# pmorenoz/HetMOGP

Measured on AMD Instinct MI355X. Metric: ELBO-steps/sec (one step = ELBO + all parameter gradients), higher is better.
Workload: dtype f64

## Files before the change

### hetmogp_amd/csrc/common.h

```cpp
#pragma once
#include <hip/hip_runtime.h>
#include <stdint.h>
#include <string>

#define HMOGP_WAVE 64
#ifndef HMOGP_POTRF_NB
#define HMOGP_POTRF_NB 32
#endif

typedef double f64x4 __attribute__((ext_vector_type(4)));
typedef double f64x2 __attribute__((ext_vector_type(2)));

struct HipError {
  hipError_t code;
  const char* what;
  const char* file;
  int line;
};
#define HIP_TRY(expr)                                          \
  do {                                                         \
    hipError_t _e = (expr);                                    \
    if (_e != hipSuccess) throw HipError{_e, #expr, __FILE__, __LINE__}; \
  } while (0)

__device__ __forceinline__ double wave_sum(double v) {
#pragma unroll
  for (int o = 32; o > 0; o >>= 1) v += __shfl_xor(v, o, 64);
  return v;
}

__device__ __forceinline__ double block_sum(double v, double* scratch) {
  v = wave_sum(v);
  const int lane = threadIdx.x & 63, w = threadIdx.x >> 6, nw = (blockDim.x + 63) >> 6;
  __syncthreads();
  if (lane == 0) scratch[w] = v;
  __syncthreads();
  double r = 0.0;
  if (threadIdx.x == 0)
    for (int i = 0; i < nw; ++i) r += scratch[i];
  return r;
}

struct GemmArgs {
  const double* A = nullptr;
  const double* B = nullptr;
  double* C = nullptr;
  const double* kscale = nullptr;
  int M = 0, N = 0, K = 0;
  int lda = 0, ldb = 0, ldc = 0;
  long long sA = 0, sB = 0, sC = 0, sS = 0;
  double alpha = 1.0, beta = 0.0;
  int nbatch = 1;
  int M_last = 0, N_last = 0, K_last = 0;
  int nouter = 1;
  long long oA = 0, oB = 0, oC = 0, oS = 0;
  int ksplit = 1;
  long long sSplit = 0;
  int a_kmajor = 0, b_kmajor = 1;
  int lower_only = 0;
  int diag_balance = 1;
  int role = 0;
  double* fs_part = nullptr;
  const double* fs_a = nullptr;
  const double* fs_x = nullptr;
  const double* fs_z = nullptr;
  const double* fs_ell = nullptr;
  int fs_ldz = 0, fs_P = 1, fs_hyper = 0;
  long long fs_sPart = 0, fs_sA = 0, fs_sZ = 0;
  int store_c = 1;
  int fs_sq = 0;
  const double* fs_k = nullptr;
  const double* c_src = nullptr;
  int c_sub = 0;
  int a_tri = 0, b_tri = 0;
  const int* win = nullptr;
  long long win_stride = 0;
};
void launch_combine_parts(const double* part, int tiles, long long n, double* p, double* c, double* pt, double* ct,
                          hipStream_t s, int nb = 1, long long sPart = 0, long long ldn = 0);
void launch_gemm_f64(const GemmArgs& g, hipStream_t stream);
bool gemm_rowpass_eligible(const GemmArgs& g);
void launch_gemm_rowpass(const GemmArgs& g, hipStream_t stream);
int launch_gemm_rowpass_or_general(const GemmArgs& g, hipStream_t stream);
bool gemm_rowpass_would_take(const GemmArgs& g);
constexpr int GEMM_MAX_FWD_PARTS = 4;
bool gemm_small_eligible(const GemmArgs& g);
void launch_gemm_small(const GemmArgs& g, hipStream_t stream);

void launch_potrf_batched(double* A, int Q, int M, int* d_info, double* dscr, hipStream_t stream, int panel_begin = 0,
                          int panel_end = -1);
void launch_trtri_batched(const double* L, double* Linv, double* tmp, int Q, int M, hipStream_t stream, bool linv_is_zero = false);
void launch_ltl_batched(const double* Linv, double* Out, int Q, int M, hipStream_t stream);

void launch_fill(double* p, long long n, double v, hipStream_t stream);
void launch_unpack_tril(const double* L_flat , double* L , int Q, int M, hipStream_t s);
void launch_gemv_batched(const double* A, const double* x, double* y, int Q, int M, long long sx, int incx,
                         hipStream_t s);
```

### hetmogp_amd/csrc/engine.hip

```cpp
#include "engine_impl.h"

hipEvent_t hmogp_engine::new_event() {
  if (pool_used == pool.size()) {
    hipEvent_t e;
    HIP_TRY(hipEventCreate(&e));
    pool.push_back(e);
  }
  return pool[pool_used++];
}

void hmogp_engine::collect_spans() {
  static const bool dbg = getenv("HMOGP_DEBUG_TIMELINE") != nullptr;
  for (auto& s : spans) {
    float f = 0.f;
    if (hipEventElapsedTime(&f, s.a, s.b) == hipSuccess) ms[s.cat] += f;
    if (dbg) {
      float t0 = 0.f;
      if (hipEventElapsedTime(&t0, ev_begin0, s.a) == hipSuccess)
        std::fprintf(stderr, "[hmogp timeline] cat %d  start %9.3f ms  dur %9.3f ms\n", s.cat, t0, f);
    }
  }
  spans.clear();
  pool_used = 0;
}

hmogp_engine::~hmogp_engine() {
  drop_graphs();
  comm_destroy();
  for (auto e : pool) (void)hipEventDestroy(e);
  if (h_info2) (void)hipHostFree(h_info2);
  if (ev_ng) (void)hipEventDestroy(ev_ng);
  if (h_small) (void)hipHostFree(h_small);
  for (auto e : {ev_begin0, ev_begin1, ev_fin0, ev_fin1, ev_fork, ev_gsk, ev_zero, ev_info, ev_S, ev_join, ev_col, ev_kuf, ev_params, ev_ua, ev_qu})
    if (e) (void)hipEventDestroy(e);
  if (hstage) (void)hipHostFree(hstage);
  if (h_info) (void)hipHostFree(h_info);
  if (h_cond) (void)hipHostFree(h_cond);
  if (ev_cond) (void)hipEventDestroy(ev_cond);
  if (st2_own) (void)hipStreamDestroy(st2_own);
  if (st3_own) (void)hipStreamDestroy(st3_own);
  if (st) (void)hipStreamDestroy(st);
}

void hmogp_engine::init(const hmogp_config* c) {
  if (!c || c->abi_version != HMOGP_ABI_VERSION) throw EngineError{HMOGP_E_INVALID, "bad config / ABI version"};
  T = c->T, Q = c->Q, M = c->M, P = c->P, Df = c->Df, device = c->device;
  if (T < 1 || Q < 1 || M < 1 || Df < 1) throw EngineError{HMOGP_E_INVALID, "T, Q, M, Df must be >= 1"};
  if (P < 1 || P > 4) throw EngineError{HMOGP_E_INVALID, "input dimension P must be 1..4"};
  if (Q > HMOGP_MAXQ) throw EngineError{HMOGP_E_INVALID, "Q exceeds HMOGP_MAXQ (8)"};
  if (c->chunk_rows > 0) {
    chunk = c->chunk_rows;
  } else {
    const long long fit = (64LL << 30) / (16LL * Q * M);
    chunk = std::max<long long>(4096, std::min<long long>(1048576, fit / 1024 * 1024));
  }
  use_windows = (c->flags & HMOGP_CFG_EXACT_ZERO_WINDOWS) != 0;
  cache_kuu = (c->flags & HMOGP_CFG_CACHE_KUU) != 0;
  no_small = (c->flags & HMOGP_CFG_NO_SMALL_PATH) != 0;
  strict = strict_cfg = (c->flags & HMOGP_CFG_STRICT_QF) != 0;
  if (strict && use_windows) throw EngineError{HMOGP_E_INVALID, "HMOGP_CFG_STRICT_QF and HMOGP_CFG_EXACT_ZERO_WINDOWS exclude each other"};
  if (c->flags & ~(HMOGP_CFG_EXACT_ZERO_WINDOWS | HMOGP_CFG_CACHE_KUU | HMOGP_CFG_NO_SMALL_PATH | HMOGP_CFG_STRICT_QF))
    throw EngineError{HMOGP_E_INVALID, "unknown bits in hmogp_config.flags"};
  quirks = c->quirks;
  if (quirks & ~HMOGP_QUIRKS_REFERENCE) throw EngineError{HMOGP_E_INVALID, "unknown bits in hmogp_config.quirks"};
  if (use_windows && M > 8192) throw EngineError{HMOGP_E_INVALID, "exact-zero windows support M <= 8192"};
  int ndev = 0;
  if (hipGetDeviceCount(&ndev) != hipSuccess || ndev < 1)
    throw EngineError{HMOGP_E_NO_DEVICE, "no HIP device visible (this library has no CPU path)"};
  if (device < 0 || device >= ndev) throw EngineError{HMOGP_E_NO_DEVICE, "HIP device ordinal out of range"};
  HIP_TRY(hipSetDevice(device));
  {
    int lo = 0, hi = 0;
    HIP_TRY(hipDeviceGetStreamPriorityRange(&lo, &hi));
    HIP_TRY(hipStreamCreateWithPriority(&st, hipStreamNonBlocking, hi));
    const char* cus_env = getenv("HMOGP_ST2_CUS");
    int cus = cus_env ? atoi(cus_env) : 0;
    hipDeviceProp_t prop;
    HIP_TRY(hipGetDeviceProperties(&prop, device));
    if (cus > 0 && cus < prop.multiProcessorCount) {
      std::vector<uint32_t> mask((prop.multiProcessorCount + 31) / 32, 0u);
      for (int i = 0; i < cus; ++i) mask[i / 32] |= 1u << (i % 32);
      if (hipExtStreamCreateWithCUMask(&st2, (uint32_t)mask.size(), mask.data()) != hipSuccess) st2 = nullptr;
    }
    const char* free_env = getenv("HMOGP_ST2_FREE");
    const int nfree = free_env ? atoi(free_env) : 0;
    if (!st2 && nfree > 0 && nfree < 32 && prop.multiProcessorCount == 256) {
      const char* lay = getenv("HMOGP_ST2_LAYOUT");
      const int layout = lay ? atoi(lay) : 1;
      st2_masked = true;
      std::vector<uint32_t> mask(8, 0xFFFFFFFFu);
      for (int x = 0; x < 8; ++x)
        for (int c = 32 - nfree; c < 32; ++c) {
          const int bit = layout == 0 ? x * 32 + c : c * 8 + x;
          mask[bit / 32] &= ~(1u << (bit % 32));
        }
      if (hipExtStreamCreateWithCUMask(&st2, (uint32_t)mask.size(), mask.data()) != hipSuccess) st2 = nullptr, st2_masked = false;
    }
    if (!st2) HIP_TRY(hipStreamCreateWithPriority(&st2, hipStreamNonBlocking, lo));
    HIP_TRY(hipStreamCreateWithPriority(&st3, hipStreamNonBlocking, hi));
    st2_own = st2, st3_own = st3;
  }
  for (hipEvent_t* e : {&ev_fork, &ev_gsk, &ev_zero, &ev_info, &ev_S, &ev_join, &ev_col, &ev_kuf, &ev_params, &ev_ua, &ev_qu})
    HIP_TRY(hipEventCreateWithFlags(e, hipEventDisableTiming));
  HIP_TRY(hipEventRecord(ev_qu, st));
  HIP_TRY(hipEventRecord(ev_join, st));
  for (hipEvent_t* e : {&ev_begin0, &ev_begin1, &ev_fin0, &ev_fin1}) HIP_TRY(hipEventCreate(e));
  f_index.assign(c->f_index, c->f_index + Df);
  d_index.assign(c->d_index, c->d_index + Df);
  tasks.resize(T);
  int d = 0;
  for (int t = 0; t < T; ++t) {
    Task& k = tasks[t];
    k.lik = c->lik_id[t];
    k.param = c->lik_param ? c->lik_param[t] : 0.0;
    if (k.lik == HMOGP_LIK_GAUSSIAN && !(k.param > 0.0)) k.param = 0.5;
    k.dimf = lik_dimf(k.lik, k.param);
    check_lik_param(k.lik, k.param);
    k.qparam = k.lik == HMOGP_LIK_ORDINAL ? ordinal_table(k.param).sigma : k.param;
    if (k.dimf < 1 || k.dimf > HMOGP_MAXJ) throw EngineError{HMOGP_E_INVALID, "unsupported likelihood / dim_f"};
    k.d0 = d;
    for (int j = 0; j < k.dimf; ++j, ++d)
      if (d >= Df || f_index[d] != t || d_index[d] != j)
        throw EngineError{HMOGP_E_INVALID, "f_index / d_index inconsistent with the likelihood list"};
  }
  if (d != Df) throw EngineError{HMOGP_E_INVALID, "Df does not match the likelihood list"};
  const long long MM = (long long)M * M;
  NG = 2 + Df;
  oR = MM, oDZ = MM + M, oSA = oDZ + (long long)M * P, oSL = oSA + 1, oSWK = oSA + 2;
  per_q = oSWK + Df;
  nstats = NG + Q * per_q;
  stats.ensure(sizeof(double) * nstats, true);
  nwire = NG + Q * ((long long)M * (M + 1) / 2 + (per_q - MM));
  for (int t = 0; t < T; ++t) {
    Task& k = tasks[t];
    const int J = k.dimf;
    k.nscal = 2 + 2 * Q + J + Q * J;
    std::vector<long long> off(k.nscal);
    off[0] = 0, off[1] = 1;
    for (int q = 0; q < Q; ++q) {
      off[2 + 2 * q] = NG + q * per_q + oSA;
      off[3 + 2 * q] = NG + q * per_q + oSL;
      for (int j = 0; j < J; ++j) off[2 + 2 * Q + J + q * J + j] = NG + q * per_q + oSWK + k.d0 + j;
    }
    for (int j = 0; j < J; ++j) off[2 + 2 * Q + j] = 2 + k.d0 + j;
    k.offsets.ensure(sizeof(long long) * k.nscal);
    HIP_TRY(hipMemcpy(k.offsets.p, off.data(), sizeof(long long) * k.nscal, hipMemcpyHostToDevice));
  }
  const size_t mmq = sizeof(double) * MM * Q;
  for (DevBuf* b : {&Kuu, &Luu, &Kuui, &L, &S, &KiS, &KSK, &C, &Ctri, &Sqi, &tmpA, &tmpB, &HK, &G, &GSK, &dKmm, &dLdS}) b->ensure(mmq, true);
  oJit = 2 * Q + 2 * Q * Df, oW0 = oJit + Q, oBs = oW0 + Q * Df, oSeq = oBs + T;
  n_small = oSeq + 1;
  auto even = [](long long n) { return (n + 1) & ~1LL; };
  const long long nZ = (long long)M * Q * P, nmu = (long long)M * Q, nL = ((long long)M * (M + 1) / 2) * Q;
  oZ = even(n_small), oMu = oZ + even(nZ), oLf = oMu + even(nmu), n_params = oLf + even(nL);
  dparams.ensure(sizeof(double) * n_params);
// ... 448 lines not shown
```

### hetmogp_amd/csrc/engine_impl.h

```cpp
#pragma once
#include <algorithm>
#include <cmath>
#include <cstdio>
#include <cstdlib>
#include <cstring>
#include <string>
#include <vector>

#include <chrono>
#include <thread>

#include <dlfcn.h>
#include <hip/hip_runtime.h>
extern "C" {
typedef struct ncclComm* ncclComm_t;
}
namespace hm_nccl {
struct UniqueId { char internal[128]; };
enum : int { Success = 0, InProgress = 7, DataDouble = 8, OpSum = 0 };
using GetUniqueId = int (*)(UniqueId*);
using CommInitRank = int (*)(ncclComm_t*, int, UniqueId, int);
using CommDestroy = int (*)(ncclComm_t);
using CommAbort = int (*)(ncclComm_t);
using CommGetAsyncError = int (*)(ncclComm_t, int*);
// ... 166 lines not shown
  double* h_small = nullptr;
  long long n_small = 0, oZ = 0, oMu = 0, oLf = 0, n_params = 0, oJit = 0, oW0 = 0, oBs = 0, oSeq = 0;
  int eval_seq = 0;
  DevBuf Kuu, Luu, Kuui, L, S, KiS, KSK, C, Ctri, Sqi, tmpA, tmpB, HK, G, GSK, dKmm, dLdS;
  DevBuf a, Kr, gmu, gL, klout, rowout, dinfo, djit, dscr;
  long long ws_rows = 0;
  DevBuf Kh, Pt, vp, vc, vpt, vct, valpha, vbeta, valpha0, vbeta0;
  DevBuf colred;
  DevBuf stats, wire, slabs, colpart, quadpart, fwdpart, winrow, wincol, winhit, Xws, dstage;
  long long nwire = 0;
  int* h_info = nullptr;
  double* hstage = nullptr;
  size_t hstage_cap = 0;
  bool began = false, evaluated = false;
  bool qu_resident = false;
  DevBuf ad_gms_m, ad_sms_m, ad_step_m, ad_pend_m, ad_gms_L, ad_sms_L, ad_step_L, ad_pend_L;

  struct Span {
    hipEvent_t a, b;
    int cat;
  };
  std::vector<hipEvent_t> pool;
  size_t pool_used = 0;
  std::vector<Span> spans;
  double ms[NCAT] = {0};
  long long launches[NCAT] = {0};
  hipEvent_t ev_begin0 = nullptr, ev_begin1 = nullptr, ev_fin0 = nullptr, ev_fin1 = nullptr;
  bool st2_masked = false;
  hipStream_t st2_own = nullptr, st3_own = nullptr;
  bool small_mode = false;
  bool small_path = false, small_veto = false, small_info_pending = false, info_early = false;
  double* hstage_dev = nullptr;
  bool small_rows = false;
  DevBuf smallslab;
  struct RetryRegular {};
  struct SmallGraph {
    std::vector<long long> key;
    hipGraph_t graph = nullptr;
    hipGraphExec_t exec = nullptr;
  };
  std::vector<SmallGraph> graphs;
  std::vector<std::vector<long long>> warm_keys;
  long long graph_replays = 0, graph_captures = 0;
  void drop_graphs(bool keep_warm = false);
  std::vector<long long> graph_key(const hmogp_params* p) const;
  bool graph_step(const hmogp_params* p, hmogp_outputs* out);
  bool graphs_broken = false, via_graph = false;
  std::vector<long long> pending_warm;
  void mark_warm();
  hipStream_t st2 = nullptr;
  hipStream_t st3 = nullptr;
  hipEvent_t ev_qu = nullptr;
  hipEvent_t ev_fork = nullptr, ev_gsk = nullptr, ev_zero = nullptr, ev_info = nullptr, ev_S = nullptr, ev_join = nullptr, ev_col = nullptr, ev_kuf = nullptr, ev_params = nullptr,
             ev_ua = nullptr;

  hipEvent_t new_event();
  struct Scope {
    hmogp_engine* e;
    Span s;
    hipStream_t stream;
    bool on_;
    Scope(hmogp_engine* eng, int cat, int nlaunch, hipStream_t on = nullptr) : e(eng), stream(on ? on : eng->st) {
      static const bool off = getenv("HMOGP_NO_SPANS") != nullptr;
      on_ = !off && (!eng->small_mode || cat == CAT_EXCHANGE);
      s.cat = cat;
      e->launches[cat] += nlaunch;
      if (!on_) return;
      s.a = e->new_event();
      s.b = e->new_event();
      (void)hipEventRecord(s.a, stream);
    }
    ~Scope() {
      if (!on_) return;
      (void)hipEventRecord(s.b, stream);
      e->spans.push_back(s);
    }
  };
  void collect_spans();

  ncclComm_t comm = nullptr;
  int comm_ranks = 1, comm_rank = 0;
  bool exchanged = false;

  void comm_init(int nranks, int rank, const void* id);
  void comm_destroy();
  void comm_abort();
  void wait_exchanged();
  void exchange();

  ~hmogp_engine();

  double* Hq(int q) { return stats.d() + NG + q * per_q; }

  void init(const hmogp_config* c);

  void set_task_data(int t, const double* X, const double* Y, long long N);

  void ensure_workspace(long long rows);

  long long ws_strict_rows = 0;
  void ensure_strict_workspace();

  void upload_params(const hmogp_params* p, bool enqueue = true);

  void mm(const double* A, bool a_k, const double* B, bool b_k, double* Cc, double alpha = 1.0, long long sA = -1,
          int lda = -1, hipStream_t stream = nullptr, int a_tri = 0, int b_tri = 0, bool lower_only = false) {
    GemmArgs g;
// ... 72 lines not shown
```

### hetmogp_amd/csrc/engine_rows.hip

```cpp
#include "engine_impl.h"

void hmogp_engine::u_algebra_small() {
  Scope sc(this, CAT_MM, 1);
  kuu_key_valid = false;
  if (!h_info) HIP_TRY(hipHostMalloc((void**)&h_info, sizeof(int) * HMOGP_MAXQ, hipHostMallocDefault));
  for (int q = 0; q < Q; ++q)
    if (rung[q] == -2) rung[q] = -1;
  if (!pools.empty()) {
    stage_pool_inputs(pools[0], st);
    if (!small_rows) kuf_pool(pools[0], st);
    kuf_prefetched = true;
    HIP_TRY(hipEventRecord(ev_kuf, st));
  }
  SmallU u;
  u.M = M, u.Q = Q, u.P = P, u.ldz = Q * P;
  u.Z = dZ.d(), u.var = dvar.d(), u.ell = dell.d(), u.jit = dsmall.d() + oJit, u.mu = dmu.d(), u.Lflat = dLflat.d();
  u.Kuu = Kuu.d(), u.Luu = Luu.d(), u.Kuui = Kuui.d(), u.L = L.d(), u.S = S.d(), u.KiS = KiS.d(), u.KSK = KSK.d(), u.C = C.d();
  u.Ctri = Ctri.d(), u.Sqi = Sqi.d(), u.a = a.d(), u.klout = klout.d(), u.info = dinfo.as<int>(), u.flag = dinfo.as<int>() + HMOGP_MAXQ;
  u.seq = dsmall.d() + oSeq;
  u.zero = stats.d(), u.nzero = nstats;
  launch_u_small(u, st);
  if (info_early) HIP_TRY(hipMemcpyAsync(h_info, dinfo.p, sizeof(int) * Q, hipMemcpyDeviceToHost, st));
  small_info_pending = true;
  HIP_TRY(hipEventRecord(ev_join, st));
// ... 216 lines not shown
    Scope sc(this, CAT_FWD, 2);
    GemmArgs g;
    g.A = Ah.d(), g.lda = M, g.a_kmajor = 0, g.sA = sK;
    g.B = Bt, g.ldb = M, g.b_kmajor = 1, g.sB = MM, g.b_tri = +1;
    g.C = Pt.d(), g.ldc = M, g.sC = sK;
    g.M = (int)n, g.N = M, g.K = M;
    g.nbatch = Q;
    g.role = 1;
    const int tiles = (M + 127) / 128;
    g.fs_part = fwdpart.d(), g.fs_sPart = 4LL * FWD_PARTS * tiles * ldn, g.fs_sq = 1, g.store_c = 0;
    static const bool t2_env = [] {
      const char* e = getenv("HMOGP_STRICT_T2");
      return !(e && e[0] == '0');
    }();
    if (t2_env && gemm_rowpass_would_take(g)) {
      const int nparts = launch_gemm_rowpass_or_general(g, st);
      launch_combine_parts(fwdpart.d(), nparts * tiles, n, nullptr, vct.d(), nullptr, nullptr, st, Q, g.fs_sPart, ldn);
      t2_fused = true;
    } else {
      rows_gemm(Ah.d(), Bt, 1, +1, Pt.d());
    }
  }
  StrictRows sr;
  sr.M = M, sr.Q = Q, sr.P = P, sr.ldz = Q * P, sr.n = n, sr.ldn = ldn, sr.sK = sK, sr.sZ = P;
  sr.Kh = Kh.d(), sr.Ah = Ah.d(), sr.Tt = Pt.d(), sr.Pt = Pt.d(), sr.mu = dmu.d(), sr.w3 = strict_two ? nullptr : w3.d(), sr.a = a.d();
  sr.X = X, sr.Z = dZ.d(), sr.ell = dell.d();
  sr.p = vp.d(), sr.c = vc.d(), sr.pg = vpg.d(), sr.cg = vcg.d(), sr.pt = nullptr, sr.ct = nullptr;
  sr.phase = 0;
  sr.t2 = t2_fused ? vct.d() : nullptr;
  {
    Scope sc(this, CAT_STRICT_STATS, 1);
    if (stats_fused && t2_fused)
      launch_trsm_stats_combine(trsmpart.d(), ts.sPart, ldn, 4, n, Q, vct.d(), vp.d(), vc.d(), ldn, st);
    else
      launch_strict_rowstats(sr, st);
  }
  sr.t2 = nullptr;
  if (!grads) return;
  static const bool p1_env = [] {
    const char* e = getenv("HMOGP_STRICT_P1");
    return !(e && e[0] == '0');
  }();
  {
    GemmArgs g;
    g.A = Ah.d(), g.lda = M, g.a_kmajor = 0, g.sA = sK;
    g.B = Bp, g.ldb = M, g.b_kmajor = 1, g.sB = MM;
    g.C = Pt.d(), g.ldc = M, g.sC = sK;
    g.M = (int)n, g.N = M, g.K = M;
    g.nbatch = Q;
    g.role = 1;
    const int tiles = (M + 127) / 128;
    g.fs_part = fwdpart.d(), g.fs_sPart = 4LL * FWD_PARTS * tiles * ldn, g.fs_a = a.d(), g.fs_sA = M, g.fs_k = Kh.d();
    if (p1_env && gemm_rowpass_would_take(g)) {
      {
        Scope sc(this, CAT_FWD, 1);
        launch_gemm_rowpass_or_general(g, st);
      }
      Scope sc(this, CAT_STRICT_STATS, 1);
      launch_combine_parts(fwdpart.d(), 4 * tiles, n, vpg.d(), vcg.d(), nullptr, nullptr, st, Q, g.fs_sPart, ldn);
      return;
    }
  }
  {
    Scope sc(this, CAT_FWD, 1);
    rows_gemm(Ah.d(), Bp, 1, 0, Pt.d());
  }
  Scope sc(this, CAT_STRICT_STATS, 1);
  sr.phase = 1;
  sr.pt = sr.ct = nullptr;
  launch_strict_rowstats(sr, st);
}

void hmogp_engine::row_pass() {
  const long long MM = (long long)M * M;
  const int ldz = Q * P;
  const bool want_hyper = (group_mask & (HMOGP_GROUP_HYPER | HMOGP_GROUP_Z)) != 0;
  const bool want_z = (group_mask & HMOGP_GROUP_Z) != 0;
  const long long ldn = ws_rows;
  if (!kuf_prefetched) HIP_TRY(hipMemsetAsync(stats.p, 0, sizeof(double) * nstats, st));
  const int tiles = (M + 127) / 128;
  const long long wtiles = (ws_rows + 127) / 128;
  const long long sK = ldn * M;
  const int ncb = (M + 127) / 128;
  for (auto& pl : pools) {
    const long long n = pl.back().off + pl.back().n;
    int* rw = use_windows ? winrow.as<int>() : nullptr;
    int* cw = use_windows ? wincol.as<int>() : nullptr;
    const double* X = tasks[pl[0].t].X.d() + pl[0].r0 * P;
    const bool prefetched = &pl == &pools[0] && kuf_prefetched;
    if (pl.size() > 1) {
      if (!prefetched) stage_pool_inputs(pl, st);
      X = Xws.d();
    }
    if (!prefetched && !small_rows) kuf_pool(pl, st);
    const long long sPart = 4LL * FWD_PARTS * tiles * ldn;
    const long long clen = (long long)M * (2 + P);
    static const bool col_sl_env = [] {
      const char* e = getenv("HMOGP_COL_SL");
      return !(e && e[0] == '0');
    }();
    const bool col_sl = want_hyper && !small_rows && col_sl_env;
    const long long csplit = col_split(n);
    const long long nsp = (n + csplit - 1) / csplit;

    auto quad_segment = [&](const Seg& sg) {
      Task& k = tasks[sg.t];
      QuadArgs qa;
      qa.lik = k.lik, qa.lik_param = k.qparam, qa.dimf = k.dimf, qa.Q = Q, qa.N = sg.n;
      qa.y = k.quad_y() + sg.r0;
      qa.yaux = k.Yaux.p ? k.Yaux.d() + sg.r0 : nullptr;
      qa.p = vp.d() + sg.off, qa.c = vc.d() + sg.off;
      const bool row_sl = want_hyper && !col_sl;
// ... 95 lines not shown
      const bool row_sl = want_hyper && !col_sl;
      qm.p = vp.d(), qm.c = vc.d(), qm.pt = row_sl ? vpt.d() : nullptr, qm.ct = row_sl ? vct.d() : nullptr;
      qm.Wd = dW.d(), qm.W0d = dsmall.d() + oW0, qm.kapd = dkap.d(), qm.vard = dvar.d(), qm.scale_base = dsmall.d() + oBs;
      qm.quirks = quirks;
      qm.alpha = valpha.d(), qm.beta = vbeta.d(), qm.alpha0 = valpha0.d(), qm.beta0 = vbeta0.d(), qm.partials = quadpart.d();
      long long part = 0;
      for (size_t i = 0; i < pl.size(); ++i) {
        const Seg& sg = pl[i];
        Task& k = tasks[sg.t];
        QuadSeg& g = qm.seg[i];
        g.lik = k.lik, g.dimf = k.dimf, g.d0 = k.d0, g.t = sg.t, g.lik_param = k.qparam, g.N = sg.n, g.off = sg.off;
        g.y = k.quad_y() + sg.r0, g.yaux = k.Yaux.p ? k.Yaux.d() + sg.r0 : nullptr;
        auto& r = qred.s[qred.nseg++];
        r.part = quadpart.d() + part, r.nrows = quad_blocks(k.lik, sg.n), r.nscal = k.nscal, r.off = k.offsets.as<long long>();
        part += r.nrows * k.nscal;
      }
      if (quad_multi || quad_multi_specialised(qm)) {
        Scope sc(this, CAT_QUAD, quad_multi ? 1 : 2);
        launch_quad_multi(qm, st);
        if (!quad_multi) launch_reduce_rows_multi(qred, stats.d(), st);
      } else {
        Scope sc(this, CAT_QUAD, 2 * (int)pl.size());
        for (auto& sg : pl) quad_segment(sg);
      }
    } else {
      Scope sc(this, CAT_QUAD, 2 * (int)pl.size());
      for (auto& sg : pl) quad_segment(sg);
    }
    if (small_rows) {
      Scope sc(this, CAT_GRAM, 2);
      launch_small_bwd(sr, st, quad_multi ? &qred : nullptr);
      continue;
    }
    colstats_rows(0, n, 0);
    {
      const int ksplit = use_windows ? std::min(8, gram_ksplit(n, M)) : gram_ksplit(n, M);
      slabs.ensure(sizeof(double) * MM * ksplit * Q, true);
      GemmArgs g;
      g.A = strict ? Ah.d() : Kh.d(), g.lda = M, g.a_kmajor = 1, g.sA = sK;
      g.B = g.A, g.ldb = M, g.b_kmajor = 1, g.sB = sK;
      g.kscale = vbeta.d(), g.sS = ldn;
      g.C = slabs.d(), g.ldc = M, g.sC = MM * ksplit;
      g.M = g.N = M, g.K = (int)n;
      g.nbatch = Q;
      g.lower_only = 1;
      g.ksplit = ksplit, g.sSplit = MM;
      g.role = 2;
      static const int bal = [] {
        const char* e = getenv("HMOGP_DIAG_BALANCE");
        return e ? atoi(e) : 1;
      }();
      g.diag_balance = bal;
      g.win = cw, g.win_stride = 2 * ncb;
      {
        Scope sc(this, CAT_GRAM, 1);
        launch_gemm_rowpass_or_general(g, st);
      }
      {
        Scope sc(this, CAT_COLSTATS, 1, st2);
        launch_reduce_slabs(colpart.d(), (int)nsp, clen, (long long)M * (1 + P), Hq(0) + oR, true, st2, Q, nsp * clen, per_q);
        if (col_sl) {
          launch_reduce_slabs(colpart.d() + (long long)M * (1 + P), (int)nsp, clen, M, colred.d(), false, st2, Q, nsp * clen, M);
          launch_sum_cols(colred.d(), Q, M, Hq(0) + oSL, per_q, st2);
        }
      }
      HIP_TRY(hipEventRecord(ev_col, st2));
      Scope sc2(this, CAT_COLSTATS, 1);
      launch_reduce_slabs_lower(slabs.d(), ksplit, M, Hq(0), true, st, Q, MM * ksplit, per_q);
    }
    HIP_TRY(hipStreamWaitEvent(st, ev_col, 0));
  }
}
```

### hetmogp_amd/csrc/gemm_rowpass.hip

```cpp
#include <cstdlib>

#include "common.h"

namespace {

constexpr int BM = 128, BN = 128, BK = 16, W = 8, NT = W * 64;
constexpr int KM_LD = 144, RM_LD = 18, TILE_DOUBLES = BK * KM_LD;
constexpr int NB = 2, WN = 32, NWN = 4;

struct Tile {
  double a[2][TILE_DOUBLES];
  double b[2][TILE_DOUBLES];
};

__device__ __forceinline__ int diag_wm(int w) { return (0x4B >> w) & 1; }
__device__ __forceinline__ int diag_wn(int w) { return (0x7E84 >> (2 * w)) & 3; }

template <int ROLE, bool FOLD = false>
__device__ __forceinline__ void rowpass_tile(const GemmArgs& g, int tiles_n, int ti, int tj, int split, Tile& lds, double* epi_a,
                                             int* hwinfo = nullptr) {
  const int batch = blockIdx.z;
  const int M = g.M, N = g.N, K = g.K;
  const int i0 = ti * BM, j0 = tj * BN;
  if (i0 >= M || j0 >= N) return;
  int wlo = 0;
  if (ROLE == 1 && g.b_tri > 0) wlo = j0;
  const int ksteps = (K - wlo + BK - 1) / BK;
  const int per = (ksteps + g.ksplit - 1) / g.ksplit;
  const int kbeg = wlo + split * per * BK;
  const int kend = min(K, kbeg + per * BK);

  const double* __restrict__ A = g.A + (long long)batch * g.sA;
  const double* __restrict__ B = g.B + (long long)batch * g.sB;
  const double* __restrict__ S = (ROLE == 2) ? g.kscale + (long long)batch * g.sS : nullptr;
  double* __restrict__ C = g.C + (long long)batch * g.sC + (long long)split * g.sSplit;
  double* fs_part = (ROLE == 1 && g.fs_part) ? g.fs_part + (long long)batch * g.fs_sPart : nullptr;

  const int t = threadIdx.x, lane = t & 63, w = __builtin_amdgcn_readfirstlane(t >> 6);
  const int lr = lane & 15, lk = lane >> 4;
  int wm = w >> 2, wn = w & 3;
  if (FOLD && w >= 4) wn = 3 - wn;
  const int klive = FOLD ? j0 + 32 * wn : 0;
  unsigned sub = 0xFFu;
  const bool diag = ROLE == 2 && ti == tj && g.lower_only;
  if (diag && hwinfo) {
    if (lane == 0) {
      const unsigned hw = __builtin_amdgcn_s_getreg(4 | (0 << 6) | (31 << 11));
      hwinfo[w] = (int)((hw >> 4) & 3u);
      if (w == 0) hwinfo[8] = (int)((hw >> 1) & 1u);
    }
  }
  constexpr bool SWAP = (ROLE == 1);
  const int blr = SWAP ? 4 * (lr & 3) + (lr >> 2) : lr;

  f64x4 acc[4][NB];
#pragma unroll
  for (int a = 0; a < 4; ++a)
#pragma unroll
    for (int b = 0; b < NB; ++b) acc[a][b] = f64x4{0.0, 0.0, 0.0, 0.0};

  const int ar = t >> 2, ak = (t & 3) * 4, bk = t >> 5, bc = (t & 31) * 2;
  const double* pa;
  const double* pb;
  if (ROLE == 1) {
    pa = A + (long long)min(i0 + ar, M - 1) * g.lda + ak;
    pb = B + (long long)bk * g.ldb + j0 + bc;
  } else {
    pa = A + i0 + bc;
    pb = B + j0 + bc;
  }
  double ra[4], rb[4], ks = 1.0;
  auto load = [&](int k0) {
    if (ROLE == 1) {
      const f64x2 x0 = *reinterpret_cast<const f64x2*>(pa + k0), x1 = *reinterpret_cast<const f64x2*>(pa + k0 + 2);
      ra[0] = x0.x, ra[1] = x0.y, ra[2] = x1.x, ra[3] = x1.y;
      const double* q = pb + (long long)k0 * g.ldb;
      const f64x2 y0 = *reinterpret_cast<const f64x2*>(q), y1 = *reinterpret_cast<const f64x2*>(q + 64);
      rb[0] = y0.x, rb[1] = y0.y, rb[2] = y1.x, rb[3] = y1.y;
    } else {
      const int row = k0 + bk;
      const long long off = (long long)min(row, K - 1) * g.lda;
      const f64x2 x0 = *reinterpret_cast<const f64x2*>(pa + off), x1 = *reinterpret_cast<const f64x2*>(pa + off + 64);
      ra[0] = x0.x, ra[1] = x0.y, ra[2] = x1.x, ra[3] = x1.y;
      const f64x2 y0 = *reinterpret_cast<const f64x2*>(pb + off), y1 = *reinterpret_cast<const f64x2*>(pb + off + 64);
      rb[0] = y0.x, rb[1] = y0.y, rb[2] = y1.x, rb[3] = y1.y;
      ks = (row < kend) ? S[row] : 0.0;
    }
  };
  auto stage = [&](int buf) {
    if (ROLE == 1) {
      double* sa = &lds.a[buf][ar * RM_LD + ak];
      *reinterpret_cast<f64x2*>(sa) = f64x2{ra[0], ra[1]};
      *reinterpret_cast<f64x2*>(sa + 2) = f64x2{ra[2], ra[3]};
    } else {
      double* sa = &lds.a[buf][bk * KM_LD + bc];
      *reinterpret_cast<f64x2*>(sa) = f64x2{ra[0], ra[1]};
      *reinterpret_cast<f64x2*>(sa + 64) = f64x2{ra[2], ra[3]};
#pragma unroll
      for (int i = 0; i < 4; ++i) rb[i] *= ks;
    }
    double* sb = &lds.b[buf][bk * KM_LD + bc];
    *reinterpret_cast<f64x2*>(sb) = f64x2{rb[0], rb[1]};
    *reinterpret_cast<f64x2*>(sb + 64) = f64x2{rb[2], rb[3]};
  };
  double fa[2][4], fb[2][NB];
  auto frag = [&](int buf, int kk, int s) {
    const double* fpa = (ROLE == 1) ? &lds.a[buf][(wm * 64 + lr) * RM_LD + kk * 4 + lk] : &lds.a[buf][(kk * 4 + lk) * KM_LD + wm * 64 + lr];
    const double* fpb = &lds.b[buf][(kk * 4 + lk) * KM_LD + wn * WN + blr];
#pragma unroll
    for (int i = 0; i < 4; ++i) fa[s][i] = fpa[i * 16 * (ROLE == 1 ? RM_LD : 1)];
#pragma unroll
    for (int i = 0; i < NB; ++i) fb[s][i] = fpb[i * 16];
  };
  auto mm8 = [&](int s) {
#pragma unroll
    for (int a = 0; a < 4; ++a)
#pragma unroll
      for (int b = 0; b < NB; ++b) {
        if (ROLE == 2 && !((sub >> (a * NB + b)) & 1u)) continue;
        acc[a][b] = SWAP ? __builtin_amdgcn_mfma_f64_16x16x4f64(fb[s][b], fa[s][a], acc[a][b], 0, 0, 0)
                         : __builtin_amdgcn_mfma_f64_16x16x4f64(fa[s][a], fb[s][b], acc[a][b], 0, 0, 0);
      }
  };

  int cur = 0;
  if (kbeg < kend) {
    load(kbeg);
    stage(0);
    if (kbeg + BK < kend) load(kbeg + BK);
  }
  __syncthreads();
  if (diag) {
    int role = w;
    if (hwinfo) {
      bool ok = true;
      unsigned seen = 0;
#pragma unroll
      for (int i = 0; i < 4; ++i) {
        ok = ok && hwinfo[i] == hwinfo[i + 4];
        seen |= 1u << hwinfo[i];
      }
      if (ok && seen == 0xFu) role = ((hwinfo[w] + 2 * hwinfo[8]) & 3) + (w & 4);
    }
    role = __builtin_amdgcn_readfirstlane(role);
    wm = diag_wm(role), wn = diag_wn(role);
    sub = 0;
#pragma unroll
    for (int a = 0; a < 4; ++a)
#pragma unroll
      for (int b = 0; b < NB; ++b)
        if (wn * NB + b <= wm * 4 + a) sub |= 1u << (a * NB + b);
  }
  const bool live = ROLE == 1 || sub != 0;
  if (ROLE == 2) {
    for (int k0 = kbeg; k0 < kend; k0 += BK) {
      if (k0 + BK < kend) stage(cur ^ 1);
      if (k0 + 2 * BK < kend) load(k0 + 2 * BK);
      if (live) {
#pragma unroll
        for (int kk = 0; kk < BK / 4; ++kk) {
          frag(cur, kk, 0);
          mm8(0);
        }
      }
      __syncthreads();
      cur ^= 1;
    }
  }
  if (ROLE == 1 && kbeg < kend && (!FOLD || kbeg >= klive)) frag(0, 0, 0);
#define HM_SB __builtin_amdgcn_sched_barrier(0)
  for (int k0 = kbeg; ROLE == 1 && k0 < kend; k0 += BK) {
    const bool more = k0 + BK < kend;
    const bool lv = !FOLD || k0 >= klive;
    if (lv) {
      frag(cur, 1, 1);
      HM_SB;
      mm8(0);
      HM_SB;
    }
    if (more) stage(cur ^ 1);
    if (k0 + 2 * BK < kend) load(k0 + 2 * BK);
    HM_SB;
    if (lv) {
      frag(cur, 2, 0);
      HM_SB;
      mm8(1);
      HM_SB;
      frag(cur, 3, 1);
      HM_SB;
      mm8(0);
      HM_SB;
    }
    __syncthreads();
    if (more && (!FOLD || k0 + BK >= klive)) frag(cur ^ 1, 0, 0);
    if (lv) {
      HM_SB;
      mm8(1);
      HM_SB;
    }
    cur ^= 1;
  }
#undef HM_SB

  if (ROLE == 1 && fs_part && g.fs_sq) {
#pragma unroll
    for (int a = 0; a < 4; ++a) {
      double sq = 0.0;
#pragma unroll
      for (int b = 0; b < NB; ++b)
#pragma unroll
        for (int r = 0; r < 4; ++r) sq = fma(acc[a][b][r], acc[a][b][r], sq);
      sq += __shfl_xor(sq, 16, 64);
      sq += __shfl_xor(sq, 32, 64);
      const int rl = wm * 64 + a * 16 + lr;
      if (lk == 0 && i0 + rl < M) fs_part[((long long)NWN * tiles_n + NWN * tj + wn) * M + (i0 + rl)] = sq;
    }
    if (!g.store_c) return;
  } else if (ROLE == 1 && fs_part) {
    constexpr int NCH = 2 * NB, WSTAGE = 2 * NCH * 128;
    double* flat = &lds.a[0][0];
    double* stg = flat + w * WSTAGE;
    static_assert(W * WSTAGE <= 4 * TILE_DOUBLES, "epilogue scratch fits the tile buffers");
    const int colq = j0 + wn * WN + 4 * lk;
    const double* __restrict__ Ke = g.fs_k ? g.fs_k + (long long)batch * g.sA : A;
    auto issue = [&](int a) {
      const int grow = min(i0 + wm * 64 + a * 16 + lr, M - 1);
      const double* src = Ke + (long long)grow * g.lda + colq;
      double* dst = stg + (a & 1) * (NCH * 128);
#pragma unroll
      for (int c = 0; c < NCH; ++c)
        __builtin_amdgcn_global_load_lds((const void __attribute__((address_space(1)))*)(src + (c >> 1) * 16 + (c & 1) * 2),
                                         (void __attribute__((address_space(3)))*)(dst + c * 128), 16, 0, 0);
    };
    issue(0);
    issue(1);
    if (t < 128) epi_a[t] = g.fs_a[(long long)batch * g.fs_sA + j0 + t];
    __syncthreads();
#pragma unroll
    for (int a = 0; a < 4; ++a) {
      if (a < 3) asm volatile("s_waitcnt vmcnt(4)" ::: "memory");
      else asm volatile("s_waitcnt vmcnt(0)" ::: "memory");
      const int rl = wm * 64 + a * 16 + lr;
      double sp = 0.0, sc = 0.0;
#pragma unroll
      for (int b = 0; b < NB; ++b) {
        const int cl = wn * WN + b * 16 + 4 * lk;
        const double* kp = stg + (a & 1) * (NCH * 128) + (2 * b) * 128 + 2 * lane;
        const f64x2 k01 = *reinterpret_cast<const f64x2*>(kp), k23 = *reinterpret_cast<const f64x2*>(kp + 128);
        const double kv[4] = {k01.x, k01.y, k23.x, k23.y};
        const f64x2 a01 = *reinterpret_cast<const f64x2*>(epi_a + cl), a23 = *reinterpret_cast<const f64x2*>(epi_a + cl + 2);
        const double av[4] = {a01.x, a01.y, a23.x, a23.y};
#pragma unroll
        for (int r = 0; r < 4; ++r) {
          sp += kv[r] * av[r];
          sc += acc[a][b][r] * kv[r];
        }
      }
#pragma unroll
      for (int o = 16; o <= 32; o <<= 1) {
        sp += __shfl_xor(sp, o, 64);
        sc += __shfl_xor(sc, o, 64);
      }
      if (lk == 0 && i0 + rl < M) {
        double* o = fs_part + ((long long)(NWN * tj + wn)) * M + (i0 + rl);
        const long long ss = (long long)NWN * tiles_n * M;
        o[0] = sp, o[ss] = sc;
      }
      if (a < 2) {
        asm volatile("" ::: "memory");
        issue(a + 2);
      }
    }
    if (!g.store_c) return;
  }
  if (SWAP) {
#pragma unroll
    for (int a = 0; a < 4; ++a) {
      const int row = i0 + wm * 64 + a * 16 + lr;
      if (row >= M) continue;
      double* crow = C + (long long)row * g.ldc + j0 + wn * WN + 4 * lk;
      if (g.c_sub) {
        const double* srow = g.c_src ? g.c_src + (long long)batch * g.sC + (long long)row * g.ldc + j0 + wn * WN + 4 * lk : crow;
#pragma unroll
        for (int b = 0; b < NB; ++b) {
          const f64x2 c01 = *reinterpret_cast<const f64x2*>(srow + b * 16), c23 = *reinterpret_cast<const f64x2*>(srow + b * 16 + 2);
          *reinterpret_cast<f64x2*>(crow + b * 16) = f64x2{c01.x - acc[a][b][0], c01.y - acc[a][b][1]};
          *reinterpret_cast<f64x2*>(crow + b * 16 + 2) = f64x2{c23.x - acc[a][b][2], c23.y - acc[a][b][3]};
        }
        continue;
      }
#pragma unroll
      for (int b = 0; b < NB; ++b) {
        *reinterpret_cast<f64x2*>(crow + b * 16) = f64x2{acc[a][b][0], acc[a][b][1]};
        *reinterpret_cast<f64x2*>(crow + b * 16 + 2) = f64x2{acc[a][b][2], acc[a][b][3]};
      }
    }
    return;
  }
#pragma unroll
  for (int a = 0; a < 4; ++a)
#pragma unroll
    for (int r = 0; r < 4; ++r) {
      double* crow = C + (long long)(i0 + wm * 64 + a * 16 + 4 * r + lk) * g.ldc + j0 + wn * WN + lr;
#pragma unroll
      for (int b = 0; b < NB; ++b)
        if ((sub >> (a * NB + b)) & 1u) crow[b * 16] = acc[a][b][r];
    }
}

template <int ROLE, bool PAIR>
__device__ __forceinline__ void rowpass_block(const GemmArgs& g, int tiles_n, int ntiles, Tile& lds, double* epi_a,
                                              int* hwinfo = nullptr) {

  int v = blockIdx.x, split = 0;
  int ti, tj;
  if (ROLE == 2 && g.lower_only) {
    const int T = tiles_n, noff = T * (T - 1) / 2, ks8 = (g.ksplit > 1) ? ((g.ksplit + 7) / 8) * 8 : 1, gx1 = noff * ks8;
    if (v < gx1) {
      int u = v;
      if (g.ksplit > 1) {
        const int xcd = v & 7, idx = v >> 3;
        split = (idx / noff) * 8 + xcd;
        u = idx % noff;
      }
      ti = (int)((sqrt(8.0 * (double)u + 1.0) + 1.0) * 0.5);
      while (ti * (ti + 1) / 2 <= u) ++ti;
      while (ti * (ti - 1) / 2 > u) --ti;
      tj = u - ti * (ti - 1) / 2;
    } else {
      const int u = v - gx1;
      split = u / T;
      ti = tj = u - split * T;
    }
    if (split >= g.ksplit) return;
  } else {
    if (g.ksplit > 1) {
      const int xcd = v & 7, idx = v >> 3;
      split = (idx / ntiles) * 8 + xcd;
      v = idx % ntiles;
      if (split >= g.ksplit) return;
    } else if ((ntiles & 7) == 0) {
      const int cpx = ntiles >> 3;
      v = (v & 7) * cpx + (v >> 3);
    }
    const int tcols = PAIR ? tiles_n / 2 : tiles_n;
    ti = v / tcols;
    tj = v - ti * tcols;
  }
  rowpass_tile<ROLE, PAIR>(g, tiles_n, ti, tj, split, lds, epi_a, hwinfo);
  if (PAIR) {
    __syncthreads();
    rowpass_tile<ROLE, PAIR>(g, tiles_n, ti, tiles_n - 1 - tj, split, lds, epi_a);
  }
}

template <int ROLE>
__global__ __launch_bounds__(NT, 4) void rowpass_gemm_kernel(GemmArgs g, int tiles_n, int ntiles) {
  __shared__ __attribute__((aligned(16))) Tile lds;
  __shared__ __attribute__((aligned(16))) double epi_a[ROLE == 1 ? 128 : 2];
  __shared__ int hwinfo[ROLE == 2 ? 16 : 1];
  rowpass_block<ROLE, false>(g, tiles_n, ntiles, lds, epi_a, (ROLE == 2 && g.diag_balance) ? hwinfo : nullptr);
}
__global__ __launch_bounds__(NT, 4) void rowpass_fold_pair_kernel(GemmArgs g, int tiles_n, int ntiles) {
  __shared__ __attribute__((aligned(16))) Tile lds;
  __shared__ __attribute__((aligned(16))) double epi_a[128];
  rowpass_block<1, true>(g, tiles_n, ntiles, lds, epi_a);
}

bool aligned16(const void* p) { return (((uintptr_t)p) & 15) == 0; }

}

bool gemm_rowpass_eligible(const GemmArgs& g) {
  const bool sub = g.role == 1 && g.alpha == -1.0 && g.beta == 1.0 && !g.fs_part && g.b_tri == 0 && g.store_c;
  if (g.nouter != 1 || (!sub && (g.alpha != 1.0 || g.beta != 0.0)) || g.win || g.M_last || g.N_last || g.K_last || g.a_tri) return false;
  if ((g.lda & 1) || (g.ldb & 1) || (g.ldc & 1) || !aligned16(g.A) || !aligned16(g.B) || !aligned16(g.C)) return false;
  if (g.c_src && (!sub || !aligned16(g.c_src))) return false;
  if (g.fs_k && (g.role != 1 || !g.fs_part || g.fs_sq || !aligned16(g.fs_k))) return false;
  if ((g.sA & 1) || (g.sB & 1) || (g.sC & 1) || (g.sSplit & 1)) return false;
  if (g.role == 1)
    return !g.a_kmajor && g.b_kmajor && !g.lower_only && g.ksplit == 1 && !g.kscale && g.b_tri >= 0 && (g.N % BN) == 0 &&
           (g.K % BK) == 0 && (g.K == g.N || sub) && g.K >= BK && g.M >= 1;
  if (g.role == 2)
    return g.a_kmajor && g.b_kmajor && g.kscale && g.b_tri == 0 && g.M == g.N && (g.N % BN) == 0 &&
           g.lda == g.ldb && g.K >= 1;
  return false;
}

void launch_gemm_rowpass(const GemmArgs& g_in, hipStream_t stream) {
  GemmArgs g = g_in;
  g.c_sub = (g.role == 1 && g.alpha == -1.0 && g.beta == 1.0) ? 1 : 0;
  const int tiles_m = (g.M + BM - 1) / BM, tiles_n = (g.N + BN - 1) / BN;
  const int ntiles = g.lower_only ? tiles_m * (tiles_m + 1) / 2 : tiles_m * tiles_n;
  const int gx = (g.ksplit > 1) ? ntiles * ((g.ksplit + 7) / 8) * 8 : ntiles;
  dim3 grid(gx, 1, g.nbatch);
  if (g.role == 1) {
    const int pair = (g.b_tri > 0 && g.ksplit == 1 && tiles_n >= 2 && (tiles_n & 1) == 0) ? 1 : 0;
    if (pair) {
      grid.x = tiles_m * (tiles_n / 2);
      hipLaunchKernelGGL(rowpass_fold_pair_kernel, grid, dim3(NT), 0, stream, g, tiles_n, (int)grid.x);
    } else {
      hipLaunchKernelGGL((rowpass_gemm_kernel<1>), grid, dim3(NT), 0, stream, g, tiles_n, ntiles);
    }
  } else {
    hipLaunchKernelGGL((rowpass_gemm_kernel<2>), grid, dim3(NT), 0, stream, g, tiles_n, ntiles);
  }
}

static bool rowpass_enabled() {
  static const bool enabled = [] {
    const char* e = getenv("HMOGP_ROWPASS");
    return !(e && e[0] == '0');
  }();
  return enabled;
}
bool gemm_rowpass_would_take(const GemmArgs& g) { return rowpass_enabled() && gemm_rowpass_eligible(g); }

int launch_gemm_rowpass_or_general(const GemmArgs& g, hipStream_t stream) {
  const bool enabled = rowpass_enabled();
  if ((g.fs_sq || g.fs_k) && !(enabled && gemm_rowpass_eligible(g)))
    throw HipError{hipErrorInvalidValue, "fs_sq / fs_k are features of the specialised forward kernel only", __FILE__, __LINE__};
  if (enabled && gemm_rowpass_eligible(g)) {
    launch_gemm_rowpass(g, stream);
    return NWN;
  }
  if (g.role == 1 && (g.alpha != 1.0 || g.beta != 0.0)) {
    GemmArgs h = g;
    h.role = 0;
    launch_gemm_f64(h, stream);
    return 2;
  }
  launch_gemm_f64(g, stream);
  return 2;
}
```

Measured before the change: 8.348.

## Split lower-only Gram into off-diagonal and diagonal phases across streams; reduce fwd partials in LDS

The lower-only Gram GEMM is split into two launches. The off-diagonal tiles run on the main stream through a specialised full-tile kernel, and the diagonal tiles run on the secondary stream after the column reductions, joined back with an event. The forward-kernel epilogues now sum the per-wave-column row statistics in LDS before writing, so each tile writes one partial per row instead of four. This shrinks the partial buffers and the combine work. The cost is an extra launch and cross-stream sync, plus a block-wide barrier in the epilogue.

```diff
diff --git a/hetmogp_amd/csrc/common.h b/hetmogp_amd/csrc/common.h
--- a/hetmogp_amd/csrc/common.h
+++ b/hetmogp_amd/csrc/common.h
@@ -59,6 +59,8 @@
   int a_kmajor = 0, b_kmajor = 1;
   int lower_only = 0;
   int diag_balance = 1;
+  int tile_phase = 0;
+  int blk0 = 0;
   int role = 0;
   double* fs_part = nullptr;
   const double* fs_a = nullptr;
@@ -83,7 +85,7 @@
 void launch_gemm_rowpass(const GemmArgs& g, hipStream_t stream);
 int launch_gemm_rowpass_or_general(const GemmArgs& g, hipStream_t stream);
 bool gemm_rowpass_would_take(const GemmArgs& g);
-constexpr int GEMM_MAX_FWD_PARTS = 4;
+constexpr int GEMM_MAX_FWD_PARTS = 2;
 bool gemm_small_eligible(const GemmArgs& g);
 void launch_gemm_small(const GemmArgs& g, hipStream_t stream);
 
diff --git a/hetmogp_amd/csrc/engine.hip b/hetmogp_amd/csrc/engine.hip
--- a/hetmogp_amd/csrc/engine.hip
+++ b/hetmogp_amd/csrc/engine.hip
@@ -31,7 +31,7 @@
   if (h_info2) (void)hipHostFree(h_info2);
   if (ev_ng) (void)hipEventDestroy(ev_ng);
   if (h_small) (void)hipHostFree(h_small);
-  for (auto e : {ev_begin0, ev_begin1, ev_fin0, ev_fin1, ev_fork, ev_gsk, ev_zero, ev_info, ev_S, ev_join, ev_col, ev_kuf, ev_params, ev_ua, ev_qu})
+  for (auto e : {ev_begin0, ev_begin1, ev_fin0, ev_fin1, ev_fork, ev_gsk, ev_zero, ev_info, ev_S, ev_join, ev_col, ev_kuf, ev_params, ev_ua, ev_qu, ev_gdiag})
     if (e) (void)hipEventDestroy(e);
   if (hstage) (void)hipHostFree(hstage);
   if (h_info) (void)hipHostFree(h_info);
@@ -100,7 +100,7 @@
     HIP_TRY(hipStreamCreateWithPriority(&st3, hipStreamNonBlocking, hi));
     st2_own = st2, st3_own = st3;
   }
-  for (hipEvent_t* e : {&ev_fork, &ev_gsk, &ev_zero, &ev_info, &ev_S, &ev_join, &ev_col, &ev_kuf, &ev_params, &ev_ua, &ev_qu})
+  for (hipEvent_t* e : {&ev_fork, &ev_gsk, &ev_zero, &ev_info, &ev_S, &ev_join, &ev_col, &ev_kuf, &ev_params, &ev_ua, &ev_qu, &ev_gdiag})
     HIP_TRY(hipEventCreateWithFlags(e, hipEventDisableTiming));
   HIP_TRY(hipEventRecord(ev_qu, st));
   HIP_TRY(hipEventRecord(ev_join, st));
diff --git a/hetmogp_amd/csrc/engine_impl.h b/hetmogp_amd/csrc/engine_impl.h
--- a/hetmogp_amd/csrc/engine_impl.h
+++ b/hetmogp_amd/csrc/engine_impl.h
@@ -242,7 +242,7 @@
   hipStream_t st3 = nullptr;
   hipEvent_t ev_qu = nullptr;
   hipEvent_t ev_fork = nullptr, ev_gsk = nullptr, ev_zero = nullptr, ev_info = nullptr, ev_S = nullptr, ev_join = nullptr, ev_col = nullptr, ev_kuf = nullptr, ev_params = nullptr,
-             ev_ua = nullptr;
+             ev_ua = nullptr, ev_gdiag = nullptr;
 
   hipEvent_t new_event();
   struct Scope {
diff --git a/hetmogp_amd/csrc/engine_rows.hip b/hetmogp_amd/csrc/engine_rows.hip
--- a/hetmogp_amd/csrc/engine_rows.hip
+++ b/hetmogp_amd/csrc/engine_rows.hip
@@ -292,12 +292,13 @@
     const int tiles = (M + 127) / 128;
     g.fs_part = fwdpart.d(), g.fs_sPart = 4LL * FWD_PARTS * tiles * ldn, g.fs_a = a.d(), g.fs_sA = M, g.fs_k = Kh.d();
     if (p1_env && gemm_rowpass_would_take(g)) {
+      int np1 = 1;
       {
         Scope sc(this, CAT_FWD, 1);
-        launch_gemm_rowpass_or_general(g, st);
+        np1 = launch_gemm_rowpass_or_general(g, st);
       }
       Scope sc(this, CAT_STRICT_STATS, 1);
-      launch_combine_parts(fwdpart.d(), 4 * tiles, n, vpg.d(), vcg.d(), nullptr, nullptr, st, Q, g.fs_sPart, ldn);
+      launch_combine_parts(fwdpart.d(), np1 * tiles, n, vpg.d(), vcg.d(), nullptr, nullptr, st, Q, g.fs_sPart, ldn);
       return;
     }
   }
@@ -499,19 +500,38 @@
       }();
       g.diag_balance = bal;
       g.win = cw, g.win_stride = 2 * ncb;
-      {
-        Scope sc(this, CAT_GRAM, 1);
+      static const bool split_env = [] {
+        const char* e = getenv("HMOGP_GRAM_SPLIT");
+        return !(e && e[0] == '0');
+      }();
+      const bool gram_split = split_env && !strict && !use_windows && tiles >= 8 && st2 != st && gemm_rowpass_would_take(g);
+      auto col_reduce = [&] {
+        {
+          Scope sc(this, CAT_COLSTATS, 1, st2);
+          launch_reduce_slabs(colpart.d(), (int)nsp, clen, (long long)M * (1 + P), Hq(0) + oR, true, st2, Q, nsp * clen, per_q);
+          if (col_sl) {
+            launch_reduce_slabs(colpart.d() + (long long)M * (1 + P), (int)nsp, clen, M, colred.d(), false, st2, Q, nsp * clen, M);
+            launch_sum_cols(colred.d(), Q, M, Hq(0) + oSL, per_q, st2);
+          }
+        }
+        HIP_TRY(hipEventRecord(ev_col, st2));
+      };
+      if (gram_split) {
+        Scope sc(this, CAT_GRAM, 2);
+        g.tile_phase = 1;
         launch_gemm_rowpass_or_general(g, st);
-      }
-      {
-        Scope sc(this, CAT_COLSTATS, 1, st2);
-        launch_reduce_slabs(colpart.d(), (int)nsp, clen, (long long)M * (1 + P), Hq(0) + oR, true, st2, Q, nsp * clen, per_q);
-        if (col_sl) {
-          launch_reduce_slabs(colpart.d() + (long long)M * (1 + P), (int)nsp, clen, M, colred.d(), false, st2, Q, nsp * clen, M);
-          launch_sum_cols(colred.d(), Q, M, Hq(0) + oSL, per_q, st2);
+        col_reduce();
+        g.tile_phase = 2;
+        launch_gemm_rowpass_or_general(g, st2);
+        HIP_TRY(hipEventRecord(ev_gdiag, st2));
+        HIP_TRY(hipStreamWaitEvent(st, ev_gdiag, 0));
+      } else {
+        {
+          Scope sc(this, CAT_GRAM, 1);
+          launch_gemm_rowpass_or_general(g, st);
         }
-      }
-      HIP_TRY(hipEventRecord(ev_col, st2));
+        col_reduce();
+      }
       Scope sc2(this, CAT_COLSTATS, 1);
       launch_reduce_slabs_lower(slabs.d(), ksplit, M, Hq(0), true, st, Q, MM * ksplit, per_q);
     }
diff --git a/hetmogp_amd/csrc/gemm_rowpass.hip b/hetmogp_amd/csrc/gemm_rowpass.hip
--- a/hetmogp_amd/csrc/gemm_rowpass.hip
+++ b/hetmogp_amd/csrc/gemm_rowpass.hip
@@ -7,6 +7,8 @@
 constexpr int BM = 128, BN = 128, BK = 16, W = 8, NT = W * 64;
 constexpr int KM_LD = 144, RM_LD = 18, TILE_DOUBLES = BK * KM_LD;
 constexpr int NB = 2, WN = 32, NWN = 4;
+constexpr int EPI_STAGE = W * 2 * (2 * NB) * 128, EPI_RED = 2 * NWN * BM;
+static_assert(EPI_STAGE + EPI_RED <= 4 * TILE_DOUBLES, "epilogue scratch fits the tile buffers");
 
 struct Tile {
   double a[2][TILE_DOUBLES];
@@ -16,7 +18,7 @@
 __device__ __forceinline__ int diag_wm(int w) { return (0x4B >> w) & 1; }
 __device__ __forceinline__ int diag_wn(int w) { return (0x7E84 >> (2 * w)) & 3; }
 
-template <int ROLE, bool FOLD = false>
+template <int ROLE, bool FOLD = false, bool FULL = false>
 __device__ __forceinline__ void rowpass_tile(const GemmArgs& g, int tiles_n, int ti, int tj, int split, Tile& lds, double* epi_a,
                                              int* hwinfo = nullptr) {
   const int batch = blockIdx.z;
@@ -42,7 +44,7 @@
   if (FOLD && w >= 4) wn = 3 - wn;
   const int klive = FOLD ? j0 + 32 * wn : 0;
   unsigned sub = 0xFFu;
-  const bool diag = ROLE == 2 && ti == tj && g.lower_only;
+  const bool diag = ROLE == 2 && !FULL && ti == tj && g.lower_only;
   if (diag && hwinfo) {
     if (lane == 0) {
       const unsigned hw = __builtin_amdgcn_s_getreg(4 | (0 << 6) | (31 << 11));
@@ -117,7 +119,7 @@
     for (int a = 0; a < 4; ++a)
 #pragma unroll
       for (int b = 0; b < NB; ++b) {
-        if (ROLE == 2 && !((sub >> (a * NB + b)) & 1u)) continue;
+        if (ROLE == 2 && !FULL && !((sub >> (a * NB + b)) & 1u)) continue;
         acc[a][b] = SWAP ? __builtin_amdgcn_mfma_f64_16x16x4f64(fb[s][b], fa[s][a], acc[a][b], 0, 0, 0)
                          : __builtin_amdgcn_mfma_f64_16x16x4f64(fa[s][a], fb[s][b], acc[a][b], 0, 0, 0);
       }
@@ -151,7 +153,7 @@
       for (int b = 0; b < NB; ++b)
         if (wn * NB + b <= wm * 4 + a) sub |= 1u << (a * NB + b);
   }
-  const bool live = ROLE == 1 || sub != 0;
+  const bool live = ROLE == 1 || FULL || sub != 0;
   if (ROLE == 2) {
     for (int k0 = kbeg; k0 < kend; k0 += BK) {
       if (k0 + BK < kend) stage(cur ^ 1);
@@ -203,6 +205,7 @@
 #undef HM_SB
 
   if (ROLE == 1 && fs_part && g.fs_sq) {
+    double* red = &lds.a[0][0] + EPI_STAGE;
 #pragma unroll
     for (int a = 0; a < 4; ++a) {
       double sq = 0.0;
@@ -213,14 +216,22 @@
       sq += __shfl_xor(sq, 16, 64);
       sq += __shfl_xor(sq, 32, 64);
       const int rl = wm * 64 + a * 16 + lr;
-      if (lk == 0 && i0 + rl < M) fs_part[((long long)NWN * tiles_n + NWN * tj + wn) * M + (i0 + rl)] = sq;
+      if (lk == 0) red[wn * BM + rl] = sq;
+    }
+    __syncthreads();
+    if (t < BM && i0 + t < M) {
+      double s = red[t];
+#pragma unroll
+      for (int c = 1; c < NWN; ++c) s += red[c * BM + t];
+      fs_part[((long long)tiles_n + tj) * M + (i0 + t)] = s;
     }
     if (!g.store_c) return;
   } else if (ROLE == 1 && fs_part) {
     constexpr int NCH = 2 * NB, WSTAGE = 2 * NCH * 128;
     double* flat = &lds.a[0][0];
     double* stg = flat + w * WSTAGE;
-    static_assert(W * WSTAGE <= 4 * TILE_DOUBLES, "epilogue scratch fits the tile buffers");
+    static_assert(W * WSTAGE == EPI_STAGE, "the row sums sit right behind the staging areas");
+    double* red = flat + EPI_STAGE;
     const int colq = j0 + wn * WN + 4 * lk;
     const double* __restrict__ Ke = g.fs_k ? g.fs_k + (long long)batch * g.sA : A;
     auto issue = [&](int a) {
@@ -261,14 +272,21 @@
         sp += __shfl_xor(sp, o, 64);
         sc += __shfl_xor(sc, o, 64);
       }
-      if (lk == 0 && i0 + rl < M) {
-        double* o = fs_part + ((long long)(NWN * tj + wn)) * M + (i0 + rl);
-        const long long ss = (long long)NWN * tiles_n * M;
-        o[0] = sp, o[ss] = sc;
-      }
+      if (lk == 0) red[wn * BM + rl] = sp, red[(NWN + wn) * BM + rl] = sc;
       if (a < 2) {
         asm volatile("" ::: "memory");
         issue(a + 2);
+      }
+    }
+    __syncthreads();
+    if (t < 2 * BM) {
+      const int stat = t >> 7, rl = t & (BM - 1);
+      if (i0 + rl < M) {
+        const double* r = red + stat * NWN * BM + rl;
+        double s = r[0];
+#pragma unroll
+        for (int c = 1; c < NWN; ++c) s += r[c * BM];
+        fs_part[((long long)stat * tiles_n + tj) * M + (i0 + rl)] = s;
       }
     }
     if (!g.store_c) return;
@@ -304,19 +322,19 @@
       double* crow = C + (long long)(i0 + wm * 64 + a * 16 + 4 * r + lk) * g.ldc + j0 + wn * WN + lr;
 #pragma unroll
       for (int b = 0; b < NB; ++b)
-        if ((sub >> (a * NB + b)) & 1u) crow[b * 16] = acc[a][b][r];
-    }
-}
-
-template <int ROLE, bool PAIR>
+        if (FULL || ((sub >> (a * NB + b)) & 1u)) crow[b * 16] = acc[a][b][r];
+    }
+}
+
+template <int ROLE, bool PAIR, bool FULL = false>
 __device__ __forceinline__ void rowpass_block(const GemmArgs& g, int tiles_n, int ntiles, Tile& lds, double* epi_a,
                                               int* hwinfo = nullptr) {
 
-  int v = blockIdx.x, split = 0;
+  int v = blockIdx.x + (ROLE == 2 ? g.blk0 : 0), split = 0;
   int ti, tj;
   if (ROLE == 2 && g.lower_only) {
     const int T = tiles_n, noff = T * (T - 1) / 2, ks8 = (g.ksplit > 1) ? ((g.ksplit + 7) / 8) * 8 : 1, gx1 = noff * ks8;
-    if (v < gx1) {
+    if (FULL || v < gx1) {
       int u = v;
       if (g.ksplit > 1) {
         const int xcd = v & 7, idx = v >> 3;
@@ -347,7 +365,7 @@
     ti = v / tcols;
     tj = v - ti * tcols;
   }
-  rowpass_tile<ROLE, PAIR>(g, tiles_n, ti, tj, split, lds, epi_a, hwinfo);
+  rowpass_tile<ROLE, PAIR, FULL>(g, tiles_n, ti, tj, split, lds, epi_a, hwinfo);
   if (PAIR) {
     __syncthreads();
     rowpass_tile<ROLE, PAIR>(g, tiles_n, ti, tiles_n - 1 - tj, split, lds, epi_a);
@@ -360,6 +378,11 @@
   __shared__ __attribute__((aligned(16))) double epi_a[ROLE == 1 ? 128 : 2];
   __shared__ int hwinfo[ROLE == 2 ? 16 : 1];
   rowpass_block<ROLE, false>(g, tiles_n, ntiles, lds, epi_a, (ROLE == 2 && g.diag_balance) ? hwinfo : nullptr);
+}
+__global__ __launch_bounds__(NT, 4) void rowpass_gram_full_kernel(GemmArgs g, int tiles_n, int ntiles) {
+  __shared__ __attribute__((aligned(16))) Tile lds;
+  __shared__ __attribute__((aligned(16))) double epi_a[2];
+  rowpass_block<2, false, true>(g, tiles_n, ntiles, lds, epi_a);
 }
 __global__ __launch_bounds__(NT, 4) void rowpass_fold_pair_kernel(GemmArgs g, int tiles_n, int ntiles) {
   __shared__ __attribute__((aligned(16))) Tile lds;
@@ -389,6 +412,7 @@
 
 void launch_gemm_rowpass(const GemmArgs& g_in, hipStream_t stream) {
   GemmArgs g = g_in;
+  g.blk0 = 0;
   g.c_sub = (g.role == 1 && g.alpha == -1.0 && g.beta == 1.0) ? 1 : 0;
   const int tiles_m = (g.M + BM - 1) / BM, tiles_n = (g.N + BN - 1) / BN;
   const int ntiles = g.lower_only ? tiles_m * (tiles_m + 1) / 2 : tiles_m * tiles_n;
@@ -402,8 +426,18 @@
     } else {
       hipLaunchKernelGGL((rowpass_gemm_kernel<1>), grid, dim3(NT), 0, stream, g, tiles_n, ntiles);
     }
+  } else if (!g.lower_only) {
+    hipLaunchKernelGGL(rowpass_gram_full_kernel, grid, dim3(NT), 0, stream, g, tiles_n, ntiles);
   } else {
-    hipLaunchKernelGGL((rowpass_gemm_kernel<2>), grid, dim3(NT), 0, stream, g, tiles_n, ntiles);
+    const int ks8 = (g.ksplit > 1) ? ((g.ksplit + 7) / 8) * 8 : 1, gx1 = tiles_m * (tiles_m - 1) / 2 * ks8;
+    if (g.tile_phase == 1) {
+      if (gx1 == 0) return;
+      grid.x = gx1;
+      hipLaunchKernelGGL(rowpass_gram_full_kernel, grid, dim3(NT), 0, stream, g, tiles_n, ntiles);
+    } else {
+      if (g.tile_phase == 2) grid.x = gx - gx1, g.blk0 = gx1;
+      hipLaunchKernelGGL((rowpass_gemm_kernel<2>), grid, dim3(NT), 0, stream, g, tiles_n, ntiles);
+    }
   }
 }
 
@@ -420,9 +454,11 @@
   const bool enabled = rowpass_enabled();
   if ((g.fs_sq || g.fs_k) && !(enabled && gemm_rowpass_eligible(g)))
     throw HipError{hipErrorInvalidValue, "fs_sq / fs_k are features of the specialised forward kernel only", __FILE__, __LINE__};
+  if (g.tile_phase && !(enabled && gemm_rowpass_eligible(g) && g.role == 2 && g.lower_only))
+    throw HipError{hipErrorInvalidValue, "tile_phase is a feature of the specialised lower-only Gram kernel", __FILE__, __LINE__};
   if (enabled && gemm_rowpass_eligible(g)) {
     launch_gemm_rowpass(g, stream);
-    return NWN;
+    return 1;
   }
   if (g.role == 1 && (g.alpha != 1.0 || g.beta != 0.0)) {
     GemmArgs h = g;
```

After: 8.367 (median of 6 runs). About the same (+0.2%).
